# givemeone1astkiss/RNA-MPNN

Measured on AMD Instinct MI355X. Metric: nucleotides/sec (forward), k=30 RNA graphs, higher is better.
Workload: dtype bf16; 1 GPU; C2: batch=256 RNAs, n~U[100,140], k=30, default 10-layer RNAMPNN, P=T; max_len=140, weights=closed-form deterministic init (3,536,900 params), parallelism=dp1

## Files before the change

### rna-mpnn_amd/csrc/api.cpp

```cpp
#include "api_internal.h"
#include "kernels_bf16.h"

#include <cstdarg>
#include <cstdlib>
#include <cstdio>
#include <cstring>
#include <string>
#include <vector>

static thread_local char g_err[512] = "";

int fail(int code, const char* fmt, ...) {
    va_list ap;
    va_start(ap, fmt);
    vsnprintf(g_err, sizeof(g_err), fmt, ap);
    va_end(ap);
    return code;
}

extern "C" const char* rnampnn_last_error(void) { return g_err; }
extern "C" const char* rnampnn_version(void) { return "rnampnn-hip 0.1 (gfx950)"; }

static int add_raw(rnampnn_ctx* c, const std::string& key, int64_t numel) {
    RawT t{key, numel, c->raw_floats, false};
// ... 558 lines not shown
        add(r.w.p_m + Nmax * RN_D, RN_D * sizeof(bf16_t));
        add(r.w.q_e + Nmax * RN_D, RN_D * sizeof(bf16_t));
        add(r.w.q_m + Nmax * RN_D, RN_D * sizeof(bf16_t));
    } else {
        add(r.w.pq_e + Nmax * 256, 256 * sizeof(float));
        add(r.w.pq_m + Nmax * 256, 256 * sizeof(float));
    }
    if (cu_seqlens) launch_lengths_from_cu(cu_seqlens, r.pk, r.s);
    else launch_lengths(mask, r.pk, r.s);
    launch_zero_regions(z, r.s);
    return RNAMPNN_OK;
}

struct PackedOut { float* logits; float* embedding; int n_total; };
static int forward_core(Run& r, rnampnn_handle h, const RnaMpnnForwardIO* io, const PackedOut* po);

extern "C" int rnampnn_forward(rnampnn_handle h, const RnaMpnnForwardIO* io, void* ws, size_t ws_bytes, void* stream) {
    if (!io || !io->coords) return fail(RNAMPNN_ERR_BAD_ARG, "rnampnn_forward: null io/coords");
    if (io->stop_after == 0 && !io->logits && !io->embedding)
        return fail(RNAMPNN_ERR_BAD_ARG, "rnampnn_forward: logits (or embedding) output required");
    Run r;
    int rc = begin_run(r, h, io->mask, io->B, io->T, ws, ws_bytes, stream);
    if (rc) return rc;
    return forward_core(r, h, io, nullptr);
}

extern "C" int rnampnn_forward_packed(rnampnn_handle h, const float* coords_packed, const int32_t* cu_seqlens, int32_t B,
                                      int32_t N_total, int32_t T_max, int32_t T_norm, float* logits_packed,
                                      float* embedding_packed, void* ws, size_t ws_bytes, void* stream) {
    if (!coords_packed || !cu_seqlens || (!logits_packed && !embedding_packed))
        return fail(RNAMPNN_ERR_BAD_ARG, "rnampnn_forward_packed: null input or no output");
    Run r;
    int rc = begin_run(r, h, nullptr, B, T_max, ws, ws_bytes, stream, cu_seqlens, N_total);
    if (rc) return rc;
    RnaMpnnForwardIO io;
    memset(&io, 0, sizeof(io));
    io.coords = coords_packed; io.B = B; io.T = T_max; io.T_norm = T_norm;
    PackedOut po{logits_packed, embedding_packed, N_total};
    return forward_core(r, h, &io, &po);
}

static int forward_core(Run& r, rnampnn_handle h, const RnaMpnnForwardIO* io, const PackedOut* po) {
    int rc = RNAMPNN_OK;
    rnampnn_ctx* c = h;
    const RnaMpnnConfig& g = c->cfg;
    if (io->T > g.padding_len)
        return fail(RNAMPNN_ERR_T_GT_P, "max_len %d exceeds padding_len %d", io->T, g.padding_len);
    int k = g.num_res_neighbours, L = g.num_res_mpnn_layers;
    int t_norm = io->T_norm > 0 ? io->T_norm : io->T;
    if (t_norm < io->T) return fail(RNAMPNN_ERR_BAD_ARG, "T_norm %d < T %d", t_norm, io->T);
    Ws& w = r.w;
    hipStream_t s = r.s;

    launch_geom(io->coords, r.pk, t_norm, io->raw, w.raw_p, w.geom, r.fast ? w.geomh : nullptr, s);
    const bool fused_first = r.fast && io->stop_after != 1;
    {
        const Lin& l = c->raw_project;
        launch_gemm_f32(r.ntot(), r.pk.Nmax, w.raw_p, RN_RAWP, l.in_pad, nullptr, 0, 0, derp<float>(c, l.wt), rawp(c, l.b), l.out,
                        l.gelu ? 1 : 0, nullptr, 0, w.n0, RN_D, r.s);
    }
    rc = run_bert(r, c->emb, w.n0, w.n1);
    if (!rc) {
        if (fused_first)
            launch_node_update(r.pk, w.n1, nullptr, rawp(c, c->feat_gn_scale), rawp(c, c->feat_gn_shift), t_norm, w.coef, w.hA, 1,
                               node_job(c, c->mpnn[0].msg, w.p_m, w.q_m), NodeJob{}, r.s);
        else
            launch_graph_norm_packed(r.pk, w.n1, nullptr, w.hA, rawp(c, c->feat_gn_scale), rawp(c, c->feat_gn_shift), t_norm, r.s);
    }
    if (rc) return rc;
    if (launch_knn(io->coords, r.pk, t_norm, k, w.nbr, io->edge_index, s))
        return fail(RNAMPNN_ERR_UNSUPPORTED, "max_len %d too long for the LDS-resident k-NN row", io->T);
    const bool embed_first = fused_first && L >= 1 && !io->e0 && resmpnn_covers(k, false, false) && !ab_switch("RNAMPNN_EMBED_TWO_LAUNCH");
    if (embed_first) { }
    else if (r.fast)
        launch_edge_embed_bf16(r.pk, k, w.geomh, w.nbr, derp<bf16_t>(c, c->edge_embed_img), rawp(c, c->edge_embed[0].b),
                               derp<float>(c, c->edge_embed_b1p), (bf16_t*)w.e, s);
    else
        launch_edge_embed_f32(r.pk, k, w.geom, w.nbr, derp<float>(c, c->edge_embed[0].wt), rawp(c, c->edge_embed[0].b),
                              g.depth_res_edge_feature > 1 ? derp<float>(c, c->edge_embed[1].wt) : nullptr,
                              g.depth_res_edge_feature > 1 ? rawp(c, c->edge_embed[1].b) : nullptr,
                              g.depth_res_edge_feature, (float*)w.e, s);
    if (io->h0) launch_unpack_nodes(r.pk, w.hA, RN_D, RN_D, io->h0, s);
    if (io->e0) unpack_e(r, io->e0);
    if (io->stop_after == 1) { HIP_TRY(hipGetLastError()); return RNAMPNN_OK; }

    if (!fused_first) node_pq(r, c->mpnn[0].msg, w.hA, false);
    bool edge_pending = false;
    int n_fused = 0;
    for (int l = 0; l < L; ++l) {
        mpnn_step(r, edge_pending ? &c->mpnn[l - 1].edge : nullptr, &c->mpnn[l].msg, w.hA, w.hB, nullptr, l == 0 && embed_first, n_fused++ & 1);
        bool tap_e = io->tap_layer == l + 1 && io->e_layer;
        edge_pending = l + 1 < L;
        const bool need_e = edge_pending || tap_e, need_m = l + 1 < L;
        const float* gsc = rawp(c, c->mpnn[l].gn_scale);
        const float* gsh = rawp(c, c->mpnn[l].gn_shift);
        if (r.fast && (need_e || need_m)) {
            const NodeJob je = need_e ? node_job(c, c->mpnn[l].edge, w.p_e, w.q_e) : NodeJob{};
            const NodeJob jm = need_m ? node_job(c, c->mpnn[l + 1].msg, w.p_m, w.q_m) : NodeJob{};
            launch_node_update(r.pk, w.hB, nullptr, gsc, gsh, t_norm, w.coef, w.hA, (need_e && need_m) ? 2 : 1, need_e ? je : jm, jm, s);
        } else {
            launch_graph_norm_packed(r.pk, w.hB, nullptr, w.hA, gsc, gsh, t_norm, s);
            if (need_e) node_pq(r, c->mpnn[l].edge, w.hA, true);
            if (need_m) node_pq(r, c->mpnn[l + 1].msg, w.hA, false);
        }
        if (io->tap_layer == l + 1) {
            if (io->h_layer) launch_unpack_nodes(r.pk, w.hA, RN_D, RN_D, io->h_layer, s);
            if (tap_e) {
                mpnn_step(r, &c->mpnn[l].edge, nullptr, w.hA, w.hB, nullptr, false, n_fused++ & 1);
                edge_pending = false;
                unpack_e(r, io->e_layer);
            }
        }
    }
    float* raw_emb = w.n2;
    rc = run_bert(r, c->post, w.hA, w.n0);
    if (rc) return rc;
    run_ffn(r, c->raw_chain, c->raw_ffn, w.raw_p, RN_RAWP, w.n1);
    launch_graph_norm_packed(r.pk, w.n1, nullptr, w.n2, rawp(c, c->rawffn_gn_scale), rawp(c, c->rawffn_gn_shift), t_norm, s);
    if (io->h_post) launch_unpack_nodes(r.pk, w.n0, RN_D, RN_D, io->h_post, s);
    if (io->raw_emb) launch_unpack_nodes(r.pk, raw_emb, RN_D, RN_D, io->raw_emb, s);
    if (io->embedding) {
        launch_unpack_nodes_strided(r.pk, w.n0, RN_D, RN_D, io->embedding, 2 * RN_D, 0, s);
        launch_unpack_nodes_strided(r.pk, raw_emb, RN_D, RN_D, io->embedding, 2 * RN_D, RN_D, s);
    }
    if (po && po->embedding) {
        HIP_TRY(hipMemcpy2DAsync(po->embedding, 2 * RN_D * sizeof(float), w.n0, RN_D * sizeof(float), RN_D * sizeof(float),
                                 po->n_total, hipMemcpyDeviceToDevice, s));
        HIP_TRY(hipMemcpy2DAsync(po->embedding + RN_D, 2 * RN_D * sizeof(float), raw_emb, RN_D * sizeof(float),
                                 RN_D * sizeof(float), po->n_total, hipMemcpyDeviceToDevice, s));
    }
    const bool want_logits = io->logits || (po && po->logits);
    float* logits_rows = (po && po->logits) ? po->logits : w.logits_p;
    if (want_logits && run_chain(r, c->readout_chain, c->readout, w.n0, RN_D, raw_emb, RN_D, logits_rows, 4)) {
        if (io->logits) launch_unpack_nodes(r.pk, logits_rows, 4, 4, io->logits, s);
    } else if (want_logits) {
        const float* cur = nullptr;
        int ld = 0;
        float* bufs[2] = {w.s0, w.s1};
        for (size_t i = 0; i < c->readout.size(); ++i) {
            const Lin& l = c->readout[i];
            bool last = i + 1 == c->readout.size();
            float* dst = last ? logits_rows : bufs[i & 1];
            if (i == 0) gemm(r, l, w.n0, RN_D, dst, l.out, nullptr, 0, raw_emb, RN_D, RN_D);
            else gemm(r, l, cur, ld, dst, l.out);
            cur = dst; ld = l.out;
        }
        if (io->logits) launch_unpack_nodes(r.pk, logits_rows, 4, 4, io->logits, s);
    }
    HIP_TRY(hipGetLastError());
    return RNAMPNN_OK;
}

extern "C" int rnampnn_mpnn_layer(rnampnn_handle h, int32_t layer, const float* h_in, const float* e_in,
                                  const int64_t* edge_index, const float* mask, int32_t B, int32_t T, int32_t T_norm,
                                  float* msg_out, float* h_out, float* e_out, void* ws, size_t ws_bytes, void* stream) {
    if (!h_in || !e_in || !edge_index) return fail(RNAMPNN_ERR_BAD_ARG, "rnampnn_mpnn_layer: null input");
    Run r;
    int rc = begin_run(r, h, mask, B, T, ws, ws_bytes, stream);
    if (rc) return rc;
    rnampnn_ctx* c = h;
    if (layer < 0 || layer >= c->cfg.num_res_mpnn_layers) return fail(RNAMPNN_ERR_BAD_ARG, "layer %d out of range", layer);
    int k = c->cfg.num_res_neighbours;
    int t_norm = T_norm > 0 ? T_norm : T;
    Ws& w = r.w;
    hipStream_t s = r.s;
    launch_pack_nodes(r.pk, h_in, RN_D, w.hA, RN_D, s);
    launch_pack_index(r.pk, k, edge_index, w.nbr, s);
    if (r.fast) {
        launch_pack_edges(r.pk, k, e_in, w.big, s);
        launch_rows_to_efrag(w.big, r.ntot(), r.pk.Nmax, k, w.nbr, (bf16_t*)w.e, s);
    } else {
// ... 113 lines not shown
```

### rna-mpnn_amd/csrc/kernels_f32.hip

```cpp
#include "api_internal.h"
#include "bf16_core.h"
#include <cstdlib>

#define WAVE 64
static constexpr float kLEPS = 1.0e6f;

__device__ __forceinline__ float wave_sum(float v) {
#pragma unroll
    for (int o = 32; o > 0; o >>= 1) v += __shfl_xor(v, o, WAVE);
    return v;
}

__global__ void k_lengths(const float* __restrict__ mask, int B, int T, int* __restrict__ len) {
    int b = blockIdx.x;
    float s = 0.f;
    for (int t = threadIdx.x; t < T; t += WAVE) s += mask[(size_t)b * T + t];
    s = wave_sum(s);
    if (threadIdx.x == 0) len[b] = (int)(s + 0.5f);
}

__device__ __forceinline__ int block_exclusive_scan_1024(int v, int* wave_tot , int* total) {
    const int lane = threadIdx.x & 63, wave = threadIdx.x >> 6;
    int inc = v;
#pragma unroll
// ... 127 lines not shown
}

__device__ __forceinline__ void raw_features(const float* c, float* f) {
    int o = 0;
#pragma unroll
    for (int a = 0; a < 7; ++a)
#pragma unroll
        for (int b = a + 1; b < 7; ++b) {
            float dx = c[a * 3] - c[b * 3], dy = c[a * 3 + 1] - c[b * 3 + 1], dz = c[a * 3 + 2] - c[b * 3 + 2];
            f[o++] = sqrtf(dx * dx + dy * dy + dz * dz + kSEPS);
        }
    float v[5][3], nr[5], u[5][3];
#pragma unroll
    for (int a = 0; a < 5; ++a) {
#pragma unroll
        for (int d = 0; d < 3; ++d) v[a][d] = c[(a + 1) * 3 + d] - c[a * 3 + d];
        nr[a] = sqrtf(v[a][0] * v[a][0] + v[a][1] * v[a][1] + v[a][2] * v[a][2]);
        float inv = 1.0f / fmaxf(nr[a], kSEPS);
#pragma unroll
        for (int d = 0; d < 3; ++d) u[a][d] = v[a][d] * inv;
    }
#pragma unroll
    for (int a = 0; a < 4; ++a)
        f[21 + a] = (v[a][0] * v[a + 1][0] + v[a][1] * v[a + 1][1] + v[a][2] * v[a + 1][2]) / (nr[a] * nr[a + 1] + kSEPS);
    float nm[4][3];
#pragma unroll
    for (int a = 0; a < 4; ++a) {
        float x = u[a][1] * u[a + 1][2] - u[a][2] * u[a + 1][1];
        float y = u[a][2] * u[a + 1][0] - u[a][0] * u[a + 1][2];
        float z = u[a][0] * u[a + 1][1] - u[a][1] * u[a + 1][0];
        float inv = 1.0f / fmaxf(sqrtf(x * x + y * y + z * z), kSEPS);
        nm[a][0] = x * inv; nm[a][1] = y * inv; nm[a][2] = z * inv;
    }
#pragma unroll
    for (int a = 0; a < 3; ++a) f[25 + a] = nm[a + 1][0] * nm[a][0] + nm[a + 1][1] * nm[a][1] + nm[a + 1][2] * nm[a][2];
}

__device__ __forceinline__ void store_geomh(const float* g, float* __restrict__ dst) {
    float gh[RN_GEOMH];
    geomh_record(g, gh);
#pragma unroll
    for (int i = 0; i < RN_GEOMH; i += 4) *reinterpret_cast<float4*>(dst + i) = make_float4(gh[i], gh[i + 1], gh[i + 2], gh[i + 3]);
}

__device__ __forceinline__ void store_geom(const float* c, float* __restrict__ geom, float* __restrict__ geomh, size_t row) {
    float g[RN_GEOM];
    geom_record(c, g);
    float* gp = geom + row * RN_GEOM;
#pragma unroll
    for (int i = 0; i < RN_GEOM; ++i) gp[i] = g[i];
    if (geomh) store_geomh(g, geomh + row * RN_GEOMH);
}

__global__ void k_geom(const float* __restrict__ coords, PackInfo pk, int Tp, float* __restrict__ raw_out,
                       float* __restrict__ raw_p, float* __restrict__ geom, float* __restrict__ geomh) {
    int id = blockIdx.x * blockDim.x + threadIdx.x;
    if (id >= pk.B * pk.T) {
        const int b = id - pk.B * pk.T;
        if (b < pk.B && pk.len[b] == pk.T && pk.T < Tp) {
            float c[21];
#pragma unroll
            for (int i = 0; i < 21; ++i) c[i] = 0.f;
            store_geom(c, geom, geomh, (size_t)(pk.Nmax + b));
        }
        return;
    }
    int b = id / pk.T, t = id - b * pk.T;
    int n = pk.len[b];
    float c[21];
    const bool have = !pk.packed_in || t < n;
    const float* src = coords + (size_t)(pk.packed_in ? pk.cu[b] + (t < n ? t : 0) : id) * 21;
#pragma unroll
    for (int i = 0; i < 21; ++i) c[i] = have ? src[i] : 0.f;
    if (t < n) {
        int p = pk.cu[b] + t;
        pk.node_b[p] = b;
        float f[28];
        raw_features(c, f);
        float* rp = raw_p + (size_t)p * RN_RAWP;
#pragma unroll
        for (int i = 0; i < 28; ++i) rp[i] = f[i];
#pragma unroll
        for (int i = 28; i < RN_RAWP; ++i) rp[i] = 0.f;
        if (raw_out) {
            float* ro = raw_out + (size_t)id * RN_RAW;
#pragma unroll
            for (int i = 0; i < 28; ++i) ro[i] = f[i];
        }
        store_geom(c, geom, geomh, (size_t)p);
    } else {
        if (raw_out) {
            float* ro = raw_out + (size_t)id * RN_RAW;
#pragma unroll
            for (int i = 0; i < 21; ++i) ro[i] = kLEPS;
#pragma unroll
            for (int i = 21; i < 28; ++i) ro[i] = 0.f;
        }
        if (t == n) store_geom(c, geom, geomh, (size_t)(pk.Nmax + b));
    }
}

void launch_geom(const float* coords, const PackInfo& pk, int Tp, float* raw_out, float* raw_p, float* geom, float* geomh, hipStream_t s) {
    int total = pk.B * (pk.T + 1);
    hipLaunchKernelGGL(k_geom, dim3((total + 63) / 64), dim3(64), 0, s, coords, pk, Tp, raw_out, raw_p, geom, geomh);
}

template <int G>
__global__ void __launch_bounds__(256) k_knn(const float* __restrict__ coords, PackInfo pk, int Tp, int k, int rows_per_block,
                                              int* __restrict__ nbr, int64_t* __restrict__ eidx) {
    extern __shared__ __attribute__((aligned(16))) float sm[];
    constexpr int GROUPS = 256 / G;
    int b = blockIdx.x;
    int n = pk.len[b];
    int T = pk.T;
    int row0 = blockIdx.y * rows_per_block;
    if (row0 >= T) return;
    int gl = threadIdx.x % G, grp = threadIdx.x / G;
    float* cen = sm;
    float* drow = sm + 3 * T + grp * T;
    if (row0 < n) {
        for (int j = threadIdx.x; j < n; j += 256) {
            const float* c = coords + (size_t)(pk.packed_in ? pk.cu[b] + j : b * T + j) * 21;
            float sx = 0.f, sy = 0.f, sz = 0.f;
#pragma unroll
            for (int a = 0; a < 7; ++a) { sx += c[a * 3]; sy += c[a * 3 + 1]; sz += c[a * 3 + 2]; }
            cen[j * 3] = sx / 7.0f; cen[j * 3 + 1] = sy / 7.0f; cen[j * 3 + 2] = sz / 7.0f;
        }
    }
    __syncthreads();
    int base = pk.cu[b];
    const int row_end = min(T, row0 + rows_per_block);
    for (int i0 = row0; i0 < row_end; i0 += GROUPS) {
        const int i = i0 + grp;
        const bool row_live = i < row_end;
        const bool real = row_live && i < n;
        if (row_live && !real) {
            if (eidx) for (int s = gl; s < k; s += G) eidx[((size_t)b * T + i) * k + s] = -1;
        }
        float cx = 0.f, cy = 0.f, cz = 0.f;
        if (real) { cx = cen[i * 3]; cy = cen[i * 3 + 1]; cz = cen[i * 3 + 2]; }
        if (real) {
            for (int j = gl; j < n; j += G) {
                float dx = __fsub_rn(cen[j * 3], cx), dy = __fsub_rn(cen[j * 3 + 1], cy), dz = __fsub_rn(cen[j * 3 + 2], cz);
                float ss = __fadd_rn(__fadd_rn(__fmul_rn(dx, dx), __fmul_rn(dy, dy)), __fmul_rn(dz, dz));
                drow[j] = (j == i) ? 3.0e38f : sqrtf(__fadd_rn(ss, kSEPS));
            }
        }
        const int nreal = real ? min(k, n - 1) : 0;
        int nmax = nreal;
#pragma unroll
        for (int o = G; o < 64; o <<= 1) nmax = max(nmax, __shfl_xor(nmax, o, 64));
        unsigned long long prev = 0ull;
        const size_t pbase = (size_t)(base + i) * k;
        const size_t obase = ((size_t)b * T + i) * k;
        if constexpr (G == 64) {
            auto wave_min = [](unsigned long long v) {
#pragma unroll
// ... 332 lines not shown
                j = j < 0 ? 0 : (j > pk.Nmax ? pk.Nmax : j);
                acc[r] = pi + pq_m[(size_t)j * 256 + 128 + c];
            }
            tile_fma(X, EH_LD, RN_D, wm.wc_t, RN_D, c, g, acc);
#pragma unroll
            for (int r = 0; r < 16; ++r) acc[r] = gelu_erf(acc[r]);
            if (wm.depth > 1) {
                __syncthreads();
#pragma unroll
                for (int r = 0; r < 16; ++r) H[(g * 16 + r) * EH_LD + c] = acc[r];
                __syncthreads();
                float bias = wm.b2[c];
#pragma unroll
                for (int r = 0; r < 16; ++r) acc[r] = bias;
                tile_fma(H, EH_LD, RN_D, wm.w2_t, RN_D, c, g, acc);
#pragma unroll
                for (int r = 0; r < 16; ++r) acc[r] = gelu_erf(acc[r]);
            }
            float sum = 0.f;
            int cnt = 0;
#pragma unroll
            for (int r = 0; r < 16; ++r) {
                int s = g * 16 + r;
                bool ok = s < k && jrow[s] >= 0;
                float m = ok ? acc[r] : 0.f;
                sum += m;
                if (msg_out && s < k) msg_out[((size_t)p * k + s) * RN_D + c] = m;
            }
            for (int s = 0; s < k; ++s) cnt += jrow[s] >= 0;
            if (g == 1) part[c] = sum;
            __syncthreads();
            if (g == 0) {
                float tot = sum + part[c];
                float denom = (float)(cnt > 0 ? cnt : 1);
                h_pre[(size_t)p * RN_D + c] = h_in[(size_t)p * RN_D + c] + tot / denom;
            }
        }
        __syncthreads();
    }
}

void launch_mpnn_f32(const PackInfo& pk, int k, bool do_edge, bool do_msg, const int* nbr, float* e,
                     const float* pq_e, const float* pq_m, MpnnW32 we, MpnnW32 wm, const float* h_in,
                     float* h_pre, float* msg_out, hipStream_t s) {
    int grid = pk.Nmax < 4096 ? pk.Nmax : 4096;
    if (do_edge && do_msg)
        hipLaunchKernelGGL((k_mpnn_f32<true, true>), dim3(grid), dim3(256), 0, s, pk, k, nbr, e, pq_e, pq_m, we, wm, h_in, h_pre, msg_out);
    else if (do_edge)
        hipLaunchKernelGGL((k_mpnn_f32<true, false>), dim3(grid), dim3(256), 0, s, pk, k, nbr, e, pq_e, pq_m, we, wm, h_in, h_pre, msg_out);
    else
        hipLaunchKernelGGL((k_mpnn_f32<false, true>), dim3(grid), dim3(256), 0, s, pk, k, nbr, e, pq_e, pq_m, we, wm, h_in, h_pre, msg_out);
}

__global__ void __launch_bounds__(256) k_graph_norm_packed(PackInfo pk, const float* __restrict__ x, const float* __restrict__ add,
        float* __restrict__ y, const float* __restrict__ scale, const float* __restrict__ shift, int t_tot) {
    __shared__ float4 red[8][32];
    __shared__ float4 stat[32];
    int b = blockIdx.x;
    int n = pk.len[b];
    if (n <= 0) return;
    const size_t base = (size_t)pk.cu[b] * RN_D;
    const int cq = threadIdx.x & 31, g = threadIdx.x >> 5;
    const float4* xb = reinterpret_cast<const float4*>(x + base) + cq;
    const float4* ab = add ? reinterpret_cast<const float4*>(add + base) + cq : nullptr;
    auto ld = [&](int r) {
        float4 v = xb[(size_t)r * 32];
        if (ab) { float4 a = ab[(size_t)r * 32]; v.x += a.x; v.y += a.y; v.z += a.z; v.w += a.w; }
        return v;
    };
    float4 s = make_float4(0.f, 0.f, 0.f, 0.f);
#pragma unroll 4
    for (int r = g; r < n; r += 8) { float4 v = ld(r); s.x += v.x; s.y += v.y; s.z += v.z; s.w += v.w; }
    red[g][cq] = s;
    __syncthreads();
    if (g == 0) {
        float4 t = red[0][cq];
#pragma unroll
        for (int i = 1; i < 8; ++i) { float4 u = red[i][cq]; t.x += u.x; t.y += u.y; t.z += u.z; t.w += u.w; }
        float inv = 1.0f / (float)n;
        stat[cq] = make_float4(t.x * inv, t.y * inv, t.z * inv, t.w * inv);
    }
    __syncthreads();
    const float4 mean = stat[cq];
    float4 ss = make_float4(0.f, 0.f, 0.f, 0.f);
#pragma unroll 4
    for (int r = g; r < n; r += 8) {
        float4 v = ld(r);
        float dx = v.x - mean.x, dy = v.y - mean.y, dz = v.z - mean.z, dw = v.w - mean.w;
        ss.x = fmaf(dx, dx, ss.x); ss.y = fmaf(dy, dy, ss.y); ss.z = fmaf(dz, dz, ss.z); ss.w = fmaf(dw, dw, ss.w);
    }
    __syncthreads();
    red[g][cq] = ss;
    __syncthreads();
    float4 t = red[0][cq];
#pragma unroll
    for (int i = 1; i < 8; ++i) { float4 u = red[i][cq]; t.x += u.x; t.y += u.y; t.z += u.z; t.w += u.w; }
    const float pad = (float)(t_tot - n), fn = (float)n;
    float4 sd;
    sd.x = sqrtf((t.x + pad * mean.x * mean.x) / fn + kSEPS); sd.y = sqrtf((t.y + pad * mean.y * mean.y) / fn + kSEPS);
    sd.z = sqrtf((t.z + pad * mean.z * mean.z) / fn + kSEPS); sd.w = sqrtf((t.w + pad * mean.w * mean.w) / fn + kSEPS);
    const float4 sc = reinterpret_cast<const float4*>(scale)[cq], sh = reinterpret_cast<const float4*>(shift)[cq];
    float4* yb = reinterpret_cast<float4*>(y + base) + cq;
#pragma unroll 4
    for (int r = g; r < n; r += 8) {
        float4 v = ld(r), o;
        o.x = (v.x - mean.x) / sd.x * sc.x + sh.x; o.y = (v.y - mean.y) / sd.y * sc.y + sh.y;
        o.z = (v.z - mean.z) / sd.z * sc.z + sh.z; o.w = (v.w - mean.w) / sd.w * sc.w + sh.w;
        yb[(size_t)r * 32] = o;
    }
}

template <int NR>
__global__ void __launch_bounds__(256) k_graph_norm_packed_reg(PackInfo pk, const float* __restrict__ x, const float* __restrict__ add,
        float* __restrict__ y, const float* __restrict__ scale, const float* __restrict__ shift, int t_tot) {
    __shared__ float4 red[8][32];
    __shared__ float4 stat[32];
    const int b = blockIdx.x;
    const int n = pk.len[b];
    if (n <= 0) return;
    const size_t base = (size_t)pk.cu[b] * RN_D;
    const int cq = threadIdx.x & 31, g = threadIdx.x >> 5;
    const float4* xb = reinterpret_cast<const float4*>(x + base) + cq;
    const float4* ab = add ? reinterpret_cast<const float4*>(add + base) + cq : nullptr;
    float4 v[NR];
#pragma unroll
    for (int i = 0; i < NR; ++i) {
        const int r = g + 8 * i, rc = r < n ? r : n - 1;
        v[i] = xb[(size_t)rc * 32];
    }
    if (ab) {
#pragma unroll
        for (int i = 0; i < NR; ++i) {
            const int r = g + 8 * i, rc = r < n ? r : n - 1;
            const float4 a = ab[(size_t)rc * 32];
            v[i].x += a.x; v[i].y += a.y; v[i].z += a.z; v[i].w += a.w;
        }
    }
    float4 s = make_float4(0.f, 0.f, 0.f, 0.f);
#pragma unroll
    for (int i = 0; i < NR; ++i)
        if (g + 8 * i < n) { s.x += v[i].x; s.y += v[i].y; s.z += v[i].z; s.w += v[i].w; }
    red[g][cq] = s;
    __syncthreads();
    if (g == 0) {
        float4 t = red[0][cq];
#pragma unroll
        for (int i = 1; i < 8; ++i) { float4 u = red[i][cq]; t.x += u.x; t.y += u.y; t.z += u.z; t.w += u.w; }
        const float inv = 1.0f / (float)n;
        stat[cq] = make_float4(t.x * inv, t.y * inv, t.z * inv, t.w * inv);
    }
    __syncthreads();
    const float4 mean = stat[cq];
    float4 ss = make_float4(0.f, 0.f, 0.f, 0.f);
#pragma unroll
    for (int i = 0; i < NR; ++i)
        if (g + 8 * i < n) {
            const float dx = v[i].x - mean.x, dy = v[i].y - mean.y, dz = v[i].z - mean.z, dw = v[i].w - mean.w;
            ss.x = fmaf(dx, dx, ss.x); ss.y = fmaf(dy, dy, ss.y); ss.z = fmaf(dz, dz, ss.z); ss.w = fmaf(dw, dw, ss.w);
        }
    __syncthreads();
    red[g][cq] = ss;
    __syncthreads();
    float4 t = red[0][cq];
#pragma unroll
    for (int i = 1; i < 8; ++i) { float4 u = red[i][cq]; t.x += u.x; t.y += u.y; t.z += u.z; t.w += u.w; }
    const float pad = (float)(t_tot - n), fn = (float)n;
    float4 sd;
    sd.x = sqrtf((t.x + pad * mean.x * mean.x) / fn + kSEPS); sd.y = sqrtf((t.y + pad * mean.y * mean.y) / fn + kSEPS);
    sd.z = sqrtf((t.z + pad * mean.z * mean.z) / fn + kSEPS); sd.w = sqrtf((t.w + pad * mean.w * mean.w) / fn + kSEPS);
    const float4 sc = reinterpret_cast<const float4*>(scale)[cq], sh = reinterpret_cast<const float4*>(shift)[cq];
    float4* yb = reinterpret_cast<float4*>(y + base) + cq;
#pragma unroll
    for (int i = 0; i < NR; ++i) {
        const int r = g + 8 * i;
        if (r < n) {
            float4 o;
            o.x = (v[i].x - mean.x) / sd.x * sc.x + sh.x; o.y = (v[i].y - mean.y) / sd.y * sc.y + sh.y;
            o.z = (v[i].z - mean.z) / sd.z * sc.z + sh.z; o.w = (v[i].w - mean.w) / sd.w * sc.w + sh.w;
            yb[(size_t)r * 32] = o;
        }
    }
}

__global__ void __launch_bounds__(256) k_graph_norm_packed_c4(PackInfo pk, const float* __restrict__ x, const float* __restrict__ add,
        float* __restrict__ y, const float* __restrict__ scale, const float* __restrict__ shift, int t_tot) {
    __shared__ float4 red[32][8];
    __shared__ float4 stat[8];
    const int b = blockIdx.x;
    const int n = pk.len[b];
    if (n <= 0) return;
    const size_t base = (size_t)pk.cu[b] * RN_D;
    const int cl = threadIdx.x & 7, g = threadIdx.x >> 3, cq = 8 * blockIdx.y + cl;
    const float4* xb = reinterpret_cast<const float4*>(x + base) + cq;
    const float4* ab = add ? reinterpret_cast<const float4*>(add + base) + cq : nullptr;
    auto ld = [&](int r) {
        float4 v = xb[(size_t)r * 32];
        if (ab) { float4 a = ab[(size_t)r * 32]; v.x += a.x; v.y += a.y; v.z += a.z; v.w += a.w; }
        return v;
    };
    auto fold = [&]() {
        float4 t = red[0][cl];
#pragma unroll
        for (int i = 1; i < 32; ++i) { const float4 u = red[i][cl]; t.x += u.x; t.y += u.y; t.z += u.z; t.w += u.w; }
        return t;
    };
    float4 s = make_float4(0.f, 0.f, 0.f, 0.f);
#pragma unroll 4
    for (int r = g; r < n; r += 32) { const float4 v = ld(r); s.x += v.x; s.y += v.y; s.z += v.z; s.w += v.w; }
    red[g][cl] = s;
    __syncthreads();
    if (g == 0) {
        const float4 t = fold();
        const float inv = 1.0f / (float)n;
        stat[cl] = make_float4(t.x * inv, t.y * inv, t.z * inv, t.w * inv);
    }
    __syncthreads();
    const float4 mean = stat[cl];
    float4 ss = make_float4(0.f, 0.f, 0.f, 0.f);
#pragma unroll 4
    for (int r = g; r < n; r += 32) {
        const float4 v = ld(r);
        const float dx = v.x - mean.x, dy = v.y - mean.y, dz = v.z - mean.z, dw = v.w - mean.w;
        ss.x = fmaf(dx, dx, ss.x); ss.y = fmaf(dy, dy, ss.y); ss.z = fmaf(dz, dz, ss.z); ss.w = fmaf(dw, dw, ss.w);
    }
    red[g][cl] = ss;
    __syncthreads();
    const float4 t = fold();
    const float pad = (float)(t_tot - n), fn = (float)n;
    float4 sd;
    sd.x = sqrtf((t.x + pad * mean.x * mean.x) / fn + kSEPS); sd.y = sqrtf((t.y + pad * mean.y * mean.y) / fn + kSEPS);
    sd.z = sqrtf((t.z + pad * mean.z * mean.z) / fn + kSEPS); sd.w = sqrtf((t.w + pad * mean.w * mean.w) / fn + kSEPS);
    const float4 sc = reinterpret_cast<const float4*>(scale)[cq], sh = reinterpret_cast<const float4*>(shift)[cq];
    float4* yb = reinterpret_cast<float4*>(y + base) + cq;
#pragma unroll 4
    for (int r = g; r < n; r += 32) {
        const float4 v = ld(r);
        float4 o;
        o.x = (v.x - mean.x) / sd.x * sc.x + sh.x; o.y = (v.y - mean.y) / sd.y * sc.y + sh.y;
        o.z = (v.z - mean.z) / sd.z * sc.z + sh.z; o.w = (v.w - mean.w) / sd.w * sc.w + sh.w;
        yb[(size_t)r * 32] = o;
    }
}

void launch_graph_norm_packed(const PackInfo& pk, const float* x, const float* add, float* y, const float* scale,
                              const float* shift, int t_tot, hipStream_t s) {
    if (pk.T <= 160) hipLaunchKernelGGL(k_graph_norm_packed_reg<20>, dim3(pk.B), dim3(256), 0, s, pk, x, add, y, scale, shift, t_tot);
    else if (pk.T <= 256) hipLaunchKernelGGL(k_graph_norm_packed_reg<32>, dim3(pk.B), dim3(256), 0, s, pk, x, add, y, scale, shift, t_tot);
    else if (pk.T <= 512) hipLaunchKernelGGL(k_graph_norm_packed, dim3(pk.B), dim3(256), 0, s, pk, x, add, y, scale, shift, t_tot);
    else hipLaunchKernelGGL(k_graph_norm_packed_c4, dim3(pk.B, 4), dim3(256), 0, s, pk, x, add, y, scale, shift, t_tot);
}

__global__ void __launch_bounds__(256) k_graph_norm_padded(const float* __restrict__ x, const float* __restrict__ mask,
        const float* __restrict__ scale, const float* __restrict__ shift, int T, int t_tot, int D, float* __restrict__ y) {
    int b = blockIdx.x;
    const float* xb = x + (size_t)b * T * D;
    const float* mb = mask + (size_t)b * T;
    float* yb = y + (size_t)b * T * D;
    for (int c = threadIdx.x; c < D; c += 256) {
        float cnt = 0.f, s = 0.f;
        for (int t = 0; t < T; ++t) { float m = mb[t]; cnt += m; s += xb[(size_t)t * D + c] * m; }
        float n = cnt == 0.f ? 1.f : cnt;
        float mean = s / n;
        float ss = 0.f;
        for (int t = 0; t < T; ++t) { float d = xb[(size_t)t * D + c] * mb[t] - mean; ss = fmaf(d, d, ss); }
        ss += (float)(t_tot - T) * mean * mean;
        float sd = sqrtf(ss / n + kSEPS);
        float sc = scale[c], sh = shift[c];
        for (int t = 0; t < T; ++t) yb[(size_t)t * D + c] = ((xb[(size_t)t * D + c] - mean) / sd * sc + sh) * mb[t];
    }
}

void launch_graph_norm_padded(const float* x, const float* mask, const float* scale, const float* shift, int B, int T,
                              int t_tot, int D, float* y, hipStream_t s) {
    hipLaunchKernelGGL(k_graph_norm_padded, dim3(B), dim3(256), 0, s, x, mask, scale, shift, T, t_tot, D, y);
}

__global__ void __launch_bounds__(256) k_gemm_f32(const int* __restrict__ ntot_p, const float* __restrict__ X, int ldx, int K1,
        const float* __restrict__ X2, int ldx2, int K2, const float* __restrict__ Wt, const float* __restrict__ bias,
        int N, int act, const float* __restrict__ res, int ldres, float* __restrict__ Y, int ldy) {
    __shared__ __attribute__((aligned(16))) float Xs[32 * EH_LD];
    int ntot = *ntot_p;
    int row0 = blockIdx.x * 32;
    if (row0 >= ntot) return;
    int col0 = blockIdx.y * 128;
    int tid = threadIdx.x, c = tid & 127, g = tid >> 7;
    int cc = col0 + c;
    int cw = cc < N ? cc : N - 1;
    float acc[16];
    float bv = bias ? bias[cw] : 0.f;
#pragma unroll
    for (int r = 0; r < 16; ++r) acc[r] = bv;
    int K = K1 + K2;
    for (int k0 = 0; k0 < K; k0 += 128) {
        int kc = min(128, K - k0);
        for (int idx = tid; idx < 32 * 32; idx += 256) {
            int r = idx >> 5, q = idx & 31;
            int kk = k0 + q * 4;
            float4 v = make_float4(0.f, 0.f, 0.f, 0.f);
            int row = row0 + r;
            if (row < ntot && q * 4 < kc) {
                if (kk < K1) v = *reinterpret_cast<const float4*>(X + (size_t)row * ldx + kk);
                else v = *reinterpret_cast<const float4*>(X2 + (size_t)row * ldx2 + (kk - K1));
// ... 249 lines not shown
```

### rna-mpnn_amd/csrc/rnampnn_internal.h

```cpp
#pragma once
#include <hip/hip_runtime.h>
#include <stdint.h>
#include <stddef.h>

#define RN_D 128
#define RN_RAW 28
#define RN_RAWP 32
#define RN_ERAW 90
#define RN_ERAWP 96
#define RN_GEOM 48
#define RN_GEOMH 64
#define RN_KMAX 32

typedef unsigned short bf16_t;

#include <mutex>
struct DevAttr { std::mutex mu; size_t have[64] = {}; };
static inline void ensure_dyn_lds(const void* fn, size_t bytes, DevAttr& st) {
    if (bytes <= 64 * 1024) return;
    int dev = 0;
    (void)hipGetDevice(&dev);
    std::lock_guard<std::mutex> g(st.mu);
    size_t& h = st.have[dev & 63];
    if (h < bytes) { (void)hipFuncSetAttribute(fn, hipFuncAttributeMaxDynamicSharedMemorySize, (int)bytes); h = bytes; }
}
#include <stdlib.h>
#include <string.h>
static inline bool ab_switch(const char* name) {
    const char* v = getenv(name);
    return v && strcmp(v, "1") == 0;
}
static inline int rn_num_cus() {
    static int cus[64] = {};
    int dev = 0;
    (void)hipGetDevice(&dev);
    int& n = cus[dev & 63];
    if (!n) {
        hipDeviceProp_t p;
        n = hipGetDeviceProperties(&p, dev) == hipSuccess && p.multiProcessorCount > 0 ? p.multiProcessorCount : 256;
    }
    return n;
}

struct PackInfo {
    int* len;
    int* cu;
    int* node_b;
    int  B, T, Nmax;
    int  packed_in;
};

struct ZeroRegions { void* ptr[8]; unsigned words[8]; int n; };
void launch_zero_regions(const ZeroRegions& z, hipStream_t s);
void launch_zero_bytes(void* ptr, size_t bytes, hipStream_t s);
void launch_copy_bytes(void* dst, const void* src, size_t bytes, hipStream_t s);
void launch_lengths(const float* mask, const PackInfo& pk, hipStream_t s);
void launch_lengths_from_cu(const int32_t* cu_seqlens, const PackInfo& pk, hipStream_t s);
void launch_geom(const float* coords, const PackInfo& pk, int Tp, float* raw_out, float* raw_p, float* geom, float* geomh, hipStream_t s);
int  launch_knn(const float* coords, const PackInfo& pk, int Tp, int k, int* nbr, int64_t* edge_index_out, hipStream_t s);
void launch_edge_embed_f32(const PackInfo& pk, int k, const float* geom, const int* nbr,
                           const float* w0t, const float* b0, const float* w1t, const float* b1, int depth,
                           float* e, hipStream_t s);
struct MpnnW32 {
    const float* wc_t;
    const float* w2_t;
    const float* b2;
    int depth;
};
void launch_mpnn_f32(const PackInfo& pk, int k, bool do_edge, bool do_msg, const int* nbr,
                     float* e, const float* pq_e, const float* pq_m, MpnnW32 we, MpnnW32 wm,
                     const float* h_in, float* h_pre, float* msg_out, hipStream_t s);
void launch_graph_norm_packed(const PackInfo& pk, const float* x, const float* add, float* y, const float* scale,
                              const float* shift, int t_tot, hipStream_t s);
void launch_graph_norm_padded(const float* x, const float* mask, const float* scale, const float* shift,
                              int B, int T, int t_tot, int D, float* y, hipStream_t s);
void launch_gemm_f32(const int* ntot, int mmax, const float* X, int ldx, int K1, const float* X2, int ldx2, int K2,
                     const float* Wt, const float* bias, int N, int act, const float* res, int ldres,
                     float* Y, int ldy, hipStream_t s);
int  launch_attention_f32(const PackInfo& pk, const float* qkv, int heads, float* out, hipStream_t s);
void launch_unpack_nodes(const PackInfo& pk, const float* src, int ld, int D, float* dst, hipStream_t s);
void launch_unpack_nodes_strided(const PackInfo& pk, const float* src, int ld, int D, float* dst, int dst_ld, int dst_col0, hipStream_t s);
void launch_pack_nodes(const PackInfo& pk, const float* src, int D, float* dst, int ld, hipStream_t s);
void launch_unpack_edges(const PackInfo& pk, int k, const float* src, const int* nbr, float* dst, hipStream_t s);
void launch_pack_edges(const PackInfo& pk, int k, const float* src, float* dst, hipStream_t s);
void launch_pack_index(const PackInfo& pk, int k, const int64_t* edge_index, int* nbr, hipStream_t s);
void launch_transpose(const float* src, int ld_src, int rows, int cols, float* dst, int ld_dst, hipStream_t s);
void launch_argmax_recovery(const float* logits, const float* mask, const int32_t* labels, int B, int T,
                            int8_t* pred, int32_t* correct, int32_t* valid, hipStream_t s);
void launch_sample(const float* logits, const float* mask, int B, int T, float temperature, int n_samples,
                   uint64_t seed, const uint64_t* seed_dev, int8_t* out, hipStream_t s);

struct rnampnn_gbdt {
    int num_trees = 0, num_class = 0, num_feature = 0, total_nodes = 0;
    float base_score = 0.f;
    int *d_off = nullptr, *d_cls = nullptr;
    int4* d_nodes = nullptr;
};
int gb_fail(int code, const char* msg);
```

Measured before the change: 14.39 million nucleotides/s.

## Fuse raw_project into geom kernel and pair final graph norms

The raw-feature projection GEMM now runs inside the geometry kernel. Three extra waves per block stage the 32x128 weight matrix in LDS, and the projection is computed right after the raw features are written. The raw FFN chain is moved ahead of the MPNN loop, and its graph norm is batched with the last layer's graph norm in a single launch that uses a z-dimension to select between two parameter sets. The goal is to remove kernel launches and one round trip of the raw features. In exchange, every geom block reloads the weight matrix, and the raw FFN's norm runs in place on its own buffer.

After: 14.49 million nucleotides/s (median of 6 runs). No clear change (+0.7%).

```diff
diff --git a/rna-mpnn_amd/csrc/api.cpp b/rna-mpnn_amd/csrc/api.cpp
--- a/rna-mpnn_amd/csrc/api.cpp
+++ b/rna-mpnn_amd/csrc/api.cpp
@@ -634,12 +634,12 @@
     Ws& w = r.w;
     hipStream_t s = r.s;
 
-    launch_geom(io->coords, r.pk, t_norm, io->raw, w.raw_p, w.geom, r.fast ? w.geomh : nullptr, s);
     const bool fused_first = r.fast && io->stop_after != 1;
     {
         const Lin& l = c->raw_project;
-        launch_gemm_f32(r.ntot(), r.pk.Nmax, w.raw_p, RN_RAWP, l.in_pad, nullptr, 0, 0, derp<float>(c, l.wt), rawp(c, l.b), l.out,
-                        l.gelu ? 1 : 0, nullptr, 0, w.n0, RN_D, r.s);
+        if (l.in_pad != RN_RAWP || l.out != RN_D) return fail(RNAMPNN_ERR_UNSUPPORTED, "raw_project is not %d -> %d", RN_RAW, RN_D);
+        launch_geom(io->coords, r.pk, t_norm, io->raw, w.raw_p, w.geom, r.fast ? w.geomh : nullptr, s, derp<float>(c, l.wt), rawp(c, l.b),
+                    l.gelu ? 1 : 0, w.n0);
     }
     rc = run_bert(r, c->emb, w.n0, w.n1);
     if (!rc) {
@@ -667,6 +667,11 @@
     if (io->stop_after == 1) { HIP_TRY(hipGetLastError()); return RNAMPNN_OK; }
 
     if (!fused_first) node_pq(r, c->mpnn[0].msg, w.hA, false);
+    run_ffn(r, c->raw_chain, c->raw_ffn, w.raw_p, RN_RAWP, w.n1);
+    float* raw_emb = w.n1;
+    const float* rsc = rawp(c, c->rawffn_gn_scale);
+    const float* rsh = rawp(c, c->rawffn_gn_shift);
+    bool raw_normed = false;
     bool edge_pending = false;
     int n_fused = 0;
     for (int l = 0; l < L; ++l) {
@@ -681,7 +686,12 @@
             const NodeJob jm = need_m ? node_job(c, c->mpnn[l + 1].msg, w.p_m, w.q_m) : NodeJob{};
             launch_node_update(r.pk, w.hB, nullptr, gsc, gsh, t_norm, w.coef, w.hA, (need_e && need_m) ? 2 : 1, need_e ? je : jm, jm, s);
         } else {
-            launch_graph_norm_packed(r.pk, w.hB, nullptr, w.hA, gsc, gsh, t_norm, s);
+            if (l + 1 == L && !need_e) {
+                launch_graph_norm_packed_pair(r.pk, w.hB, w.hA, gsc, gsh, w.n1, raw_emb, rsc, rsh, t_norm, s);
+                raw_normed = true;
+            } else {
+                launch_graph_norm_packed(r.pk, w.hB, nullptr, w.hA, gsc, gsh, t_norm, s);
+            }
             if (need_e) node_pq(r, c->mpnn[l].edge, w.hA, true);
             if (need_m) node_pq(r, c->mpnn[l + 1].msg, w.hA, false);
         }
@@ -694,11 +704,9 @@
             }
         }
     }
-    float* raw_emb = w.n2;
+    if (!raw_normed) launch_graph_norm_packed(r.pk, w.n1, nullptr, raw_emb, rsc, rsh, t_norm, s);
     rc = run_bert(r, c->post, w.hA, w.n0);
     if (rc) return rc;
-    run_ffn(r, c->raw_chain, c->raw_ffn, w.raw_p, RN_RAWP, w.n1);
-    launch_graph_norm_packed(r.pk, w.n1, nullptr, w.n2, rawp(c, c->rawffn_gn_scale), rawp(c, c->rawffn_gn_shift), t_norm, s);
     if (io->h_post) launch_unpack_nodes(r.pk, w.n0, RN_D, RN_D, io->h_post, s);
     if (io->raw_emb) launch_unpack_nodes(r.pk, raw_emb, RN_D, RN_D, io->raw_emb, s);
     if (io->embedding) {
diff --git a/rna-mpnn_amd/csrc/kernels_f32.hip b/rna-mpnn_amd/csrc/kernels_f32.hip
--- a/rna-mpnn_amd/csrc/kernels_f32.hip
+++ b/rna-mpnn_amd/csrc/kernels_f32.hip
@@ -203,57 +203,125 @@
     if (geomh) store_geomh(g, geomh + row * RN_GEOMH);
 }
 
-__global__ void k_geom(const float* __restrict__ coords, PackInfo pk, int Tp, float* __restrict__ raw_out,
-                       float* __restrict__ raw_p, float* __restrict__ geom, float* __restrict__ geomh) {
-    int id = blockIdx.x * blockDim.x + threadIdx.x;
-    if (id >= pk.B * pk.T) {
-        const int b = id - pk.B * pk.T;
-        if (b < pk.B && pk.len[b] == pk.T && pk.T < Tp) {
+template <bool PROJ>
+__global__ void __launch_bounds__(256) k_geom(const float* __restrict__ coords, PackInfo pk, int Tp, float* __restrict__ raw_out,
+        float* __restrict__ raw_p, float* __restrict__ geom, float* __restrict__ geomh, const float* __restrict__ Wt,
+        const float* __restrict__ bias, int act, float* __restrict__ n0) {
+    const int lane = threadIdx.x & 63, wave = threadIdx.x >> 6;
+    __shared__ float4 xs[PROJ ? 4 * 128 : 1];
+    __shared__ float4 wsm[PROJ ? RN_RAWP * RN_D / 4 : 1];
+    int prow = -1;
+    if (PROJ) {
+        const int id = blockIdx.x * 64 + lane;
+        if (id < pk.B * pk.T) {
+            const int b = id / pk.T, t = id - b * pk.T;
+            if (t < pk.len[b]) prow = pk.cu[b] + t;
+        }
+        if (wave != 0)
+            for (int i = threadIdx.x - 64; i < RN_RAWP * RN_D / 4; i += 192) wsm[i] = reinterpret_cast<const float4*>(Wt)[i];
+    }
+    if (wave == 0) {
+        const int id = blockIdx.x * 64 + lane;
+        if (id >= pk.B * pk.T) {
+            const int b = id - pk.B * pk.T;
+            if (b < pk.B && pk.len[b] == pk.T && pk.T < Tp) {
+                float c[21];
+#pragma unroll
+                for (int i = 0; i < 21; ++i) c[i] = 0.f;
+                store_geom(c, geom, geomh, (size_t)(pk.Nmax + b));
+            }
+        } else {
+            int b = id / pk.T, t = id - b * pk.T;
+            int n = pk.len[b];
             float c[21];
-#pragma unroll
-            for (int i = 0; i < 21; ++i) c[i] = 0.f;
-            store_geom(c, geom, geomh, (size_t)(pk.Nmax + b));
-        }
-        return;
-    }
-    int b = id / pk.T, t = id - b * pk.T;
-    int n = pk.len[b];
-    float c[21];
-    const bool have = !pk.packed_in || t < n;
-    const float* src = coords + (size_t)(pk.packed_in ? pk.cu[b] + (t < n ? t : 0) : id) * 21;
-#pragma unroll
-    for (int i = 0; i < 21; ++i) c[i] = have ? src[i] : 0.f;
-    if (t < n) {
-        int p = pk.cu[b] + t;
-        pk.node_b[p] = b;
-        float f[28];
-        raw_features(c, f);
-        float* rp = raw_p + (size_t)p * RN_RAWP;
-#pragma unroll
-        for (int i = 0; i < 28; ++i) rp[i] = f[i];
-#pragma unroll
-        for (int i = 28; i < RN_RAWP; ++i) rp[i] = 0.f;
-        if (raw_out) {
-            float* ro = raw_out + (size_t)id * RN_RAW;
-#pragma unroll
-            for (int i = 0; i < 28; ++i) ro[i] = f[i];
-        }
-        store_geom(c, geom, geomh, (size_t)p);
-    } else {
-        if (raw_out) {
-            float* ro = raw_out + (size_t)id * RN_RAW;
-#pragma unroll
-            for (int i = 0; i < 21; ++i) ro[i] = kLEPS;
-#pragma unroll
-            for (int i = 21; i < 28; ++i) ro[i] = 0.f;
-        }
-        if (t == n) store_geom(c, geom, geomh, (size_t)(pk.Nmax + b));
-    }
-}
-
-void launch_geom(const float* coords, const PackInfo& pk, int Tp, float* raw_out, float* raw_p, float* geom, float* geomh, hipStream_t s) {
+            const bool have = !pk.packed_in || t < n;
+            const float* src = coords + (size_t)(pk.packed_in ? pk.cu[b] + (t < n ? t : 0) : id) * 21;
+#pragma unroll
+            for (int i = 0; i < 21; ++i) c[i] = have ? src[i] : 0.f;
+            if (t < n) {
+                int p = pk.cu[b] + t;
+                pk.node_b[p] = b;
+                float f[28];
+                raw_features(c, f);
+                float* rp = raw_p + (size_t)p * RN_RAWP;
+#pragma unroll
+                for (int i = 0; i < 28; ++i) rp[i] = f[i];
+#pragma unroll
+                for (int i = 28; i < RN_RAWP; ++i) rp[i] = 0.f;
+                if (raw_out) {
+                    float* ro = raw_out + (size_t)id * RN_RAW;
+#pragma unroll
+                    for (int i = 0; i < 28; ++i) ro[i] = f[i];
+                }
+                store_geom(c, geom, geomh, (size_t)p);
+            } else {
+                if (raw_out) {
+                    float* ro = raw_out + (size_t)id * RN_RAW;
+#pragma unroll
+                    for (int i = 0; i < 21; ++i) ro[i] = kLEPS;
+#pragma unroll
+                    for (int i = 21; i < 28; ++i) ro[i] = 0.f;
+                }
+                if (t == n) store_geom(c, geom, geomh, (size_t)(pk.Nmax + b));
+            }
+        }
+    }
+    if (!PROJ) return;
+    __syncthreads();
+#pragma unroll
+    for (int i = 0; i < 2; ++i) {
+        const int idx = lane + 64 * i, p = __shfl(prow, 16 * wave + (idx >> 3));
+        float4 v = make_float4(0.f, 0.f, 0.f, 0.f);
+        if (p >= 0) v = *reinterpret_cast<const float4*>(raw_p + (size_t)p * RN_RAWP + 4 * (idx & 7));
+        xs[wave * 128 + idx] = v;
+    }
+    float bv[2] = {0.f, 0.f};
+    if (bias) { bv[0] = bias[lane]; bv[1] = bias[64 + lane]; }
+    __syncthreads();
+    float wr[RN_RAWP][2];
+    const float* wl = reinterpret_cast<const float*>(wsm);
+#pragma unroll
+    for (int kk = 0; kk < RN_RAWP; ++kk) { wr[kk][0] = wl[kk * RN_D + lane]; wr[kk][1] = wl[kk * RN_D + 64 + lane]; }
+#pragma unroll
+    for (int j = 0; j < 16; j += 2) {
+        const int p0 = __shfl(prow, 16 * wave + j), p1 = __shfl(prow, 16 * wave + j + 1);
+        if (p0 < 0 && p1 < 0) continue;
+        float acc[2][2] = {{bv[0], bv[1]}, {bv[0], bv[1]}};
+#pragma unroll
+        for (int kk = 0; kk < RN_RAWP; kk += 4) {
+#pragma unroll
+            for (int i = 0; i < 2; ++i) {
+                const float4 xv = xs[wave * 128 + (j + i) * 8 + (kk >> 2)];
+#pragma unroll
+                for (int q = 0; q < 2; ++q) {
+                    acc[i][q] = fmaf(xv.x, wr[kk + 0][q], acc[i][q]); acc[i][q] = fmaf(xv.y, wr[kk + 1][q], acc[i][q]);
+                    acc[i][q] = fmaf(xv.z, wr[kk + 2][q], acc[i][q]); acc[i][q] = fmaf(xv.w, wr[kk + 3][q], acc[i][q]);
+                }
+            }
+        }
+#pragma unroll
+        for (int i = 0; i < 2; ++i) {
+            const int p = i ? p1 : p0;
+            if (p < 0) continue;
+#pragma unroll
+            for (int q = 0; q < 2; ++q) {
+                float v = acc[i][q];
+                if (act == 1) v = gelu_erf(v);
+                n0[(size_t)p * RN_D + 64 * q + lane] = v;
+            }
+        }
+    }
+}
+
+void launch_geom(const float* coords, const PackInfo& pk, int Tp, float* raw_out, float* raw_p, float* geom, float* geomh, hipStream_t s,
+                 const float* proj_wt, const float* proj_bias, int proj_act, float* n0) {
     int total = pk.B * (pk.T + 1);
-    hipLaunchKernelGGL(k_geom, dim3((total + 63) / 64), dim3(64), 0, s, coords, pk, Tp, raw_out, raw_p, geom, geomh);
+    if (n0)
+        hipLaunchKernelGGL(k_geom<true>, dim3((total + 63) / 64), dim3(256), 0, s, coords, pk, Tp, raw_out, raw_p, geom, geomh, proj_wt,
+                           proj_bias, proj_act, n0);
+    else
+        hipLaunchKernelGGL(k_geom<false>, dim3((total + 63) / 64), dim3(64), 0, s, coords, pk, Tp, raw_out, raw_p, geom, geomh, nullptr,
+                           nullptr, 0, nullptr);
 }
 
 template <int G>
@@ -692,8 +760,14 @@
         hipLaunchKernelGGL((k_mpnn_f32<false, true>), dim3(grid), dim3(256), 0, s, pk, k, nbr, e, pq_e, pq_m, we, wm, h_in, h_pre, msg_out);
 }
 
-__global__ void __launch_bounds__(256) k_graph_norm_packed(PackInfo pk, const float* __restrict__ x, const float* __restrict__ add,
-        float* __restrict__ y, const float* __restrict__ scale, const float* __restrict__ shift, int t_tot) {
+struct GnSet { const float* x; const float* add; float* y; const float* scale; const float* shift; };
+#define GN_PICK_SET(a, b)                                                                          \
+    const GnSet& gn_set = blockIdx.z ? (b) : (a);                                                  \
+    const float* __restrict__ x = gn_set.x; const float* __restrict__ add = gn_set.add;            \
+    float* __restrict__ y = gn_set.y;                                                              \
+    const float* __restrict__ scale = gn_set.scale; const float* __restrict__ shift = gn_set.shift
+__global__ void __launch_bounds__(256) k_graph_norm_packed(PackInfo pk, GnSet s0, GnSet s1, int t_tot) {
+    GN_PICK_SET(s0, s1);
     __shared__ float4 red[8][32];
     __shared__ float4 stat[32];
     int b = blockIdx.x;
@@ -751,8 +825,8 @@
 }
 
 template <int NR>
-__global__ void __launch_bounds__(256) k_graph_norm_packed_reg(PackInfo pk, const float* __restrict__ x, const float* __restrict__ add,
-        float* __restrict__ y, const float* __restrict__ scale, const float* __restrict__ shift, int t_tot) {
+__global__ void __launch_bounds__(256) k_graph_norm_packed_reg(PackInfo pk, GnSet s0, GnSet s1, int t_tot) {
+    GN_PICK_SET(s0, s1);
     __shared__ float4 red[8][32];
     __shared__ float4 stat[32];
     const int b = blockIdx.x;
@@ -822,8 +896,8 @@
     }
 }
 
-__global__ void __launch_bounds__(256) k_graph_norm_packed_c4(PackInfo pk, const float* __restrict__ x, const float* __restrict__ add,
-        float* __restrict__ y, const float* __restrict__ scale, const float* __restrict__ shift, int t_tot) {
+__global__ void __launch_bounds__(256) k_graph_norm_packed_c4(PackInfo pk, GnSet s0, GnSet s1, int t_tot) {
+    GN_PICK_SET(s0, s1);
     __shared__ float4 red[32][8];
     __shared__ float4 stat[8];
     const int b = blockIdx.x;
@@ -882,12 +956,21 @@
     }
 }
 
+static void launch_graph_norm_sets(const PackInfo& pk, const GnSet& a, const GnSet& b, int sets, int t_tot, hipStream_t s) {
+    const unsigned B = pk.B, Z = sets;
+    if (pk.T <= 160) hipLaunchKernelGGL(k_graph_norm_packed_reg<20>, dim3(B, 1, Z), dim3(256), 0, s, pk, a, b, t_tot);
+    else if (pk.T <= 256) hipLaunchKernelGGL(k_graph_norm_packed_reg<32>, dim3(B, 1, Z), dim3(256), 0, s, pk, a, b, t_tot);
+    else if (pk.T <= 512) hipLaunchKernelGGL(k_graph_norm_packed, dim3(B, 1, Z), dim3(256), 0, s, pk, a, b, t_tot);
+    else hipLaunchKernelGGL(k_graph_norm_packed_c4, dim3(B, 4, Z), dim3(256), 0, s, pk, a, b, t_tot);
+}
 void launch_graph_norm_packed(const PackInfo& pk, const float* x, const float* add, float* y, const float* scale,
                               const float* shift, int t_tot, hipStream_t s) {
-    if (pk.T <= 160) hipLaunchKernelGGL(k_graph_norm_packed_reg<20>, dim3(pk.B), dim3(256), 0, s, pk, x, add, y, scale, shift, t_tot);
-    else if (pk.T <= 256) hipLaunchKernelGGL(k_graph_norm_packed_reg<32>, dim3(pk.B), dim3(256), 0, s, pk, x, add, y, scale, shift, t_tot);
-    else if (pk.T <= 512) hipLaunchKernelGGL(k_graph_norm_packed, dim3(pk.B), dim3(256), 0, s, pk, x, add, y, scale, shift, t_tot);
-    else hipLaunchKernelGGL(k_graph_norm_packed_c4, dim3(pk.B, 4), dim3(256), 0, s, pk, x, add, y, scale, shift, t_tot);
+    const GnSet a{x, add, y, scale, shift};
+    launch_graph_norm_sets(pk, a, a, 1, t_tot, s);
+}
+void launch_graph_norm_packed_pair(const PackInfo& pk, const float* x0, float* y0, const float* scale0, const float* shift0,
+                                   const float* x1, float* y1, const float* scale1, const float* shift1, int t_tot, hipStream_t s) {
+    launch_graph_norm_sets(pk, GnSet{x0, nullptr, y0, scale0, shift0}, GnSet{x1, nullptr, y1, scale1, shift1}, 2, t_tot, s);
 }
 
 __global__ void __launch_bounds__(256) k_graph_norm_padded(const float* __restrict__ x, const float* __restrict__ mask,
diff --git a/rna-mpnn_amd/csrc/rnampnn_internal.h b/rna-mpnn_amd/csrc/rnampnn_internal.h
--- a/rna-mpnn_amd/csrc/rnampnn_internal.h
+++ b/rna-mpnn_amd/csrc/rnampnn_internal.h
@@ -56,7 +56,8 @@
 void launch_copy_bytes(void* dst, const void* src, size_t bytes, hipStream_t s);
 void launch_lengths(const float* mask, const PackInfo& pk, hipStream_t s);
 void launch_lengths_from_cu(const int32_t* cu_seqlens, const PackInfo& pk, hipStream_t s);
-void launch_geom(const float* coords, const PackInfo& pk, int Tp, float* raw_out, float* raw_p, float* geom, float* geomh, hipStream_t s);
+void launch_geom(const float* coords, const PackInfo& pk, int Tp, float* raw_out, float* raw_p, float* geom, float* geomh, hipStream_t s,
+                 const float* proj_wt = nullptr, const float* proj_bias = nullptr, int proj_act = 0, float* n0 = nullptr);
 int  launch_knn(const float* coords, const PackInfo& pk, int Tp, int k, int* nbr, int64_t* edge_index_out, hipStream_t s);
 void launch_edge_embed_f32(const PackInfo& pk, int k, const float* geom, const int* nbr,
                            const float* w0t, const float* b0, const float* w1t, const float* b1, int depth,
@@ -72,6 +73,8 @@
                      const float* h_in, float* h_pre, float* msg_out, hipStream_t s);
 void launch_graph_norm_packed(const PackInfo& pk, const float* x, const float* add, float* y, const float* scale,
                               const float* shift, int t_tot, hipStream_t s);
+void launch_graph_norm_packed_pair(const PackInfo& pk, const float* x0, float* y0, const float* scale0, const float* shift0,
+                                   const float* x1, float* y1, const float* scale1, const float* shift1, int t_tot, hipStream_t s);
 void launch_graph_norm_padded(const float* x, const float* mask, const float* scale, const float* shift,
                               int B, int T, int t_tot, int D, float* y, hipStream_t s);
 void launch_gemm_f32(const int* ntot, int mmax, const float* X, int ldx, int K1, const float* X2, int ldx2, int K2,
```
